# td-kwj-zp2023/webgpu-msm-twisted-edwards

Measured on AMD Instinct MI355X. Metric: MSMs/sec at n=2^20 Twisted-Edwards BLS12 (pipelined throughput = 1000/ms_per_step; single-MSM latency in latency_ms), higher is better.
Workload: dtype u32

## Files before the change

webgpu-msm-twisted-edwards_amd/csrc/kernels.hip.hpp:

```cpp
#pragma once
#include <hip/hip_runtime.h>
#include "curve.hpp"
#include "scalar_form.hpp"

namespace te {

#define TE_BATCH_MAX 8
struct batch_ptrs { const uint4* p[TE_BATCH_MAX]; };
struct batch_slabs { uint32_t s[TE_BATCH_MAX]; };

struct digits_params {
  uint32_t half[10];
  uint32_t zero_digit;
  uint32_t sc_stride;
  uint32_t n, nst;
  int num_windows;
  int w_first, w_step, nw_local;
  uint32_t half_code, logS, P, CH, chunk_len;
};

struct pnt_slot { uint4 q[8]; };
template <bool MONT = false>
__device__ __forceinline__ void prep_points_block(uint32_t blk, uint4* __restrict__ lds, const uint4* __restrict__ pts, pnt_slot* __restrict__ recs, uint32_t n) {
  const uint32_t t = threadIdx.x, base = blk * 256u;
  const bool active = t < 256u;
  const uint32_t pieces_in = (n - base < 256u ? n - base : 256u) * 4u;
// ... 424 lines not shown
__device__ __forceinline__ bool l2_piece_of_block(uint32_t bx, const uint32_t* __restrict__ pc, uint32_t P, uint32_t overflow_pieces, uint32_t* sm, uint32_t* pj, uint32_t& p, uint32_t& j) {
  if (bx < P) { p = bx; j = 0u; return true; }
  const uint32_t t = threadIdx.x, x = bx - P;
  if (x >= overflow_pieces) return false;
  const uint32_t c = t < P ? pc[t] : 0u;
  const uint32_t ov = c ? (c + TE_L2_CAP - 1u) / TE_L2_CAP - 1u : 0u;
  uint32_t tot;
  const uint32_t ex = block_excl_scan(ov, sm, tot);
  if (x >= tot) return false;
  if (x >= ex && x < ex + ov) { pj[0] = t; pj[1] = x - ex + 1u; }
  __syncthreads();
  p = pj[0]; j = pj[1];
  __syncthreads();
  return true;
}

#define TE_COMBINE_SMALL 16u
#define TE_GIANT_RUN 256u
#define TE_SEG_INVALID 0xffffffffu
#define TE_HIST_COPIES 32u
struct plan_args {
  const uint32_t* part_start; const uint32_t* part_count; const uint32_t* seg_part_base;
  uint32_t *bucket_start, *bucket_cursor, *seg_base, *seg_bucket, *seg_lenv, *size_hist, *split_list;
  uint32_t* split_count;
  uint32_t* chunk_list;
  uint32_t seg_len, cap_w, chunk_cap;
};
struct plan_lds { uint32_t h[1024]; uint32_t sm[17]; uint32_t giant[256 * 3]; uint32_t n_giant; };
__device__ __forceinline__ uint32_t seg_plan_block(uint32_t p, uint32_t k, uint32_t cnt_in, const sort_geom& sg, const plan_args& a, plan_lds& L,
                                                   uint32_t pstart, uint32_t pcount, uint32_t sbase) {
  const uint32_t t = threadIdx.x, P = sg.P, S = sg.S, B = sg.B, seg_len = a.seg_len;
  uint32_t* const h = L.h; uint32_t* const sm = L.sm; uint32_t* const giant = L.giant;
  __syncthreads();
  for (uint32_t j = t; j < 1024u; j += 256u) h[j] = 0u;
  if (t == 0) L.n_giant = 0u;
  const bool mine = t < S;
  const uint32_t g = k * B + p * S + (mine ? t : 0u);
  const uint32_t cnt = mine ? cnt_in : 0u;
  const uint32_t nparts = mine ? max(1u, (cnt + seg_len - 1u) / seg_len) : 0u;
  uint32_t bt, bt2;
  const uint32_t ex = block_excl_scan(cnt, sm, bt);
  const uint32_t ex2 = block_excl_scan(nparts, sm, bt2);
  const uint32_t bs = pstart + ex, sb = sbase + ex2;
  if (mine) {
    a.bucket_start[g] = bs; a.bucket_cursor[g] = bs; a.seg_base[g] = sb;
    if (nparts <= TE_COMBINE_SMALL) {
      for (uint32_t part = 0; part < nparts; part++) {
        const uint32_t len = cnt > part * seg_len ? min(seg_len, cnt - part * seg_len) : 0u;
        a.seg_bucket[sb + part] = g; a.seg_lenv[sb + part] = len;
        atomicAdd(&h[min(len, 1023u)], 1u);
      }
      if (nparts > 1u) a.split_list[atomicAdd(&a.split_count[0], 1u)] = g;
    } else {
      const uint32_t j = atomicAdd(&L.n_giant, 1u);
      giant[3 * j] = g; giant[3 * j + 1] = sb; giant[3 * j + 2] = cnt;
      atomicAdd(&a.split_count[1], 1u);
    }
  }
  {
    const uint32_t first = sbase, used = bt2;
    const uint32_t cap = p + 1u == P ? (k + 1u) * a.cap_w - first : S + pcount / seg_len;
    for (uint32_t j = used + t; j < cap; j += 256u) { a.seg_bucket[first + j] = TE_SEG_INVALID; a.seg_lenv[first + j] = TE_SEG_INVALID; }
  }
  __syncthreads();
  const uint32_t ng = L.n_giant;
  for (uint32_t j = 0; j < ng; j++) {
    const uint32_t gg = giant[3 * j], sb0 = giant[3 * j + 1], c0 = giant[3 * j + 2];
    const uint32_t np = (c0 + seg_len - 1u) / seg_len;
    for (uint32_t part = t; part < np; part += 256u) {
      const uint32_t len = min(seg_len, c0 - part * seg_len);
      a.seg_bucket[sb0 + part] = gg; a.seg_lenv[sb0 + part] = len;
      atomicAdd(&h[min(len, 1023u)], 1u);
      if ((part & (TE_GIANT_RUN - 1u)) == 0) { const uint32_t ci = atomicAdd(&a.split_count[2], 1u); if (ci < a.chunk_cap) { a.chunk_list[2 * ci] = gg; a.chunk_list[2 * ci + 1] = part; } }
    }
  }
  __syncthreads();
  uint32_t* my_hist = a.size_hist + ((k * P + p) % TE_HIST_COPIES) * 1024u;
  for (uint32_t j = t; j < 1024u; j += 256u) if (h[j]) atomicAdd(&my_hist[j], h[j]);
  __syncthreads();
  return ex;
}

struct l2_args {
  const uint16_t* part_keys; const uint32_t* part_idx; const uint32_t* part_start; const uint32_t* part_count;
  uint32_t* bucket_count; uint32_t* sorted;
  uint32_t* part_ticket;
  sort_geom g; plan_args pa;
};
#define TE_L2A_LDS_WORDS (3u * 256u + 32u + TE_L2_LIST)
static_assert(sizeof(plan_lds) <= TE_L2_LIST * 4u, "the plan's LDS fits into the list area");
static_assert(TE_L2_CAP < 65536u, "k_l2_local counts a bucket's positive and negative entries in the halves of one word");
template <bool PK>
__global__ void __launch_bounds__(256, TE_L2_WAVES) k_l2_local(l2_args a) {
  __shared__ uint32_t lds[TE_L2A_LDS_WORDS];
// ... 37 lines not shown
  if (t < g.S) a.bucket_count[gb] = c0;
  const uint32_t ex = seg_plan_block(p, k, c0, g, a.pa, PL, pb, cntp, sbp);
  if (t < g.S) a.pa.bucket_cursor[gb] = pb + ex + c0;
  off_s[t] = ex; off_s[256u + t] = ex + c_pos;
  __syncthreads();
#pragma unroll
  for (int c = 0; c < 5; c++) {
    uint32_t kv[8], iv[8]; piece_group<PK>(r, c, kv, iv);
    const uint32_t e0 = ((uint32_t)c * 256u + t) * 8u;
#pragma unroll
    for (int e = 0; e < 8; e++) {
      const uint32_t pos = e0 + (uint32_t)e;
      if (pos >= head && pos < total) list[atomicAdd(&off_s[(kv[e] & 0x7fffu) + ((kv[e] >> 15) << 8)], 1u)] = iv[e] | ((kv[e] >> 15) << 31);
    }
  }
  __syncthreads();
  uint32_t* out = a.sorted + (size_t)k * g.n + pb;
  for (uint32_t s = t; s < cntp; s += 256u) out[s] = list[s];
}

#define TE_ORDER_REGS 32u
__device__ __forceinline__ void order_scatter_block(uint32_t ob, uint32_t nob, uint32_t* __restrict__ lds, const uint32_t* __restrict__ lenv, uint32_t ids,
                                                    const uint32_t* __restrict__ size_hist, uint32_t* __restrict__ rel_cursor,
                                                    uint32_t* __restrict__ order, uint32_t* __restrict__ num_segments, uint32_t max_len) {
  uint32_t* const h = lds; uint32_t* const base = lds + 1024; uint32_t* const sm = lds + 2048;
  const uint32_t per = (ids + nob - 1) / nob;
  const uint32_t lo = min(ids, ob * per), hi = min(ids, lo + per);
  const bool in_regs = per <= TE_ORDER_REGS * 256u;
  uint32_t lv[TE_ORDER_REGS];
  if (in_regs) {
#pragma unroll
    for (uint32_t j = 0; j < TE_ORDER_REGS; j++) { const uint32_t g = lo + j * 256u + threadIdx.x; lv[j] = g < hi ? lenv[g] : TE_SEG_INVALID; }
  }
  for (uint32_t j = threadIdx.x; j < 1024u; j += 256u) h[j] = 0;
  {
    uint32_t run = 0;
    for (uint32_t c = (1023u - min(max_len, 1023u)) >> 8; c < 4u; c++) {
      const uint32_t s = 1023u - (c * 256u + threadIdx.x);
      uint32_t part[TE_HIST_COPIES];
#pragma unroll
      for (uint32_t r = 0; r < TE_HIST_COPIES; r++) part[r] = size_hist[r * 1024u + s];
      uint32_t cnt_s = 0;
#pragma unroll
      for (uint32_t r = 0; r < TE_HIST_COPIES; r++) cnt_s += part[r];
      uint32_t bt;
      const uint32_t ex = block_excl_scan(cnt_s, sm, bt);
      base[s] = run + ex;
      run += bt;
    }
    if (ob == 0 && threadIdx.x == 0) *num_segments = run;
  }
  __syncthreads();
  if (in_regs) {
#pragma unroll
    for (uint32_t j = 0; j < TE_ORDER_REGS; j++) if (lv[j] != TE_SEG_INVALID) atomicAdd(&h[min(lv[j], 1023u)], 1u);
  } else {
    for (uint32_t g = lo + threadIdx.x; g < hi; g += 256u) { const uint32_t l = lenv[g]; if (l != TE_SEG_INVALID) atomicAdd(&h[min(l, 1023u)], 1u); }
  }
  __syncthreads();
  for (uint32_t j = threadIdx.x; j < 1024u; j += 256u) { base[j] += h[j] ? atomicAdd(&rel_cursor[j], h[j]) : 0u; h[j] = 0; }
  __syncthreads();
  if (in_regs) {
#pragma unroll
    for (uint32_t j = 0; j < TE_ORDER_REGS; j++) {
      if (lv[j] == TE_SEG_INVALID) continue;
      const uint32_t sz = min(lv[j], 1023u);
      order[base[sz] + atomicAdd(&h[sz], 1u)] = lo + j * 256u + threadIdx.x;
    }
  } else {
    for (uint32_t g = lo + threadIdx.x; g < hi; g += 256u) {
      const uint32_t l = lenv[g];
      if (l == TE_SEG_INVALID) continue;
      const uint32_t sz = min(l, 1023u);
      order[base[sz] + atomicAdd(&h[sz], 1u)] = g;
    }
  }
}

#define TE_PLACE_LDS_WORDS (4u * 256u + TE_L2_LIST + TE_L2_LIST / 4u + 2u + 17u)
template <bool PK>
__device__ __forceinline__ void l2_place_piece(uint32_t p, uint32_t k, uint32_t a0, uint32_t b0, uint32_t* __restrict__ lds,
                                               const uint16_t* __restrict__ part_keys, const uint32_t* __restrict__ part_idx,
                                               uint32_t* __restrict__ bucket_cursor, uint32_t* __restrict__ sorted, const sort_geom& g) {
  uint32_t* const cnt_s = lds; uint32_t* const lex_s = lds + 256; uint32_t* const off_s = lds + 512; uint32_t* const gbase_s = lds + 768;
  uint32_t* const list = lds + 1024;
  uint8_t* const list_b = reinterpret_cast<uint8_t*>(list + TE_L2_LIST);
  uint32_t* const sm = list + TE_L2_LIST + TE_L2_LIST / 4u + 2u;
  const uint32_t t = threadIdx.x, len = b0 - a0;
  const uint16_t* keys_row = part_keys + (size_t)k * g.nst; const uint32_t* idx_row = part_idx + (size_t)k * g.nst;
  uint32_t* out = sorted + (size_t)k * g.n;
  cnt_s[t] = 0u;
  __syncthreads();
  piece_regs r; uint32_t head, total;
  load_piece<PK>(keys_row, idx_row, a0, b0, t, true, r, head, total);
#pragma unroll
  for (int c = 0; c < 5; c++) {
    uint32_t kv[8], iv[8]; piece_group<PK>(r, c, kv, iv);
// ... 9 lines not shown
  }
  __syncthreads();
  off_s[t] = lex_s[t];
  gbase_s[t] -= lex_s[t];
  __syncthreads();
#pragma unroll
  for (int c = 0; c < 5; c++) {
    uint32_t kv[8], iv[8]; piece_group<PK>(r, c, kv, iv);
    const uint32_t e0 = ((uint32_t)c * 256u + t) * 8u;
#pragma unroll
    for (int e = 0; e < 8; e++) {
      const uint32_t pos = e0 + (uint32_t)e;
      if (pos >= head && pos < total) {
        const uint32_t b = kv[e] & 0x7fffu;
        const uint32_t slot = atomicAdd(&off_s[b], 1u);
        list[slot] = iv[e] | ((kv[e] >> 15) << 31); list_b[slot] = (uint8_t)b;
      }
    }
  }
  __syncthreads();
  for (uint32_t s = t; s < len; s += 256u) out[gbase_s[list_b[s]] + s] = list[s];
}

struct order_args { const uint32_t* lenv; uint32_t ids; const uint32_t* size_hist; uint32_t* rel_cursor; uint32_t* order; uint32_t* num_segments; uint32_t order_cols, max_len; };
template <bool PK>
__global__ void __launch_bounds__(256, TE_L2_WAVES) k_l2_place_order(const uint16_t* __restrict__ part_keys, const uint32_t* __restrict__ part_idx,
                                                           const uint32_t* __restrict__ part_start, const uint32_t* __restrict__ part_count,
                                                           uint32_t* __restrict__ bucket_cursor, uint32_t* __restrict__ sorted, sort_geom g, order_args oa) {
  __shared__ uint32_t lds[TE_PLACE_LDS_WORDS];
  if (blockIdx.x < oa.order_cols) {
    order_scatter_block(blockIdx.y * oa.order_cols + blockIdx.x, gridDim.y * oa.order_cols, lds, oa.lenv, oa.ids, oa.size_hist, oa.rel_cursor, oa.order, oa.num_segments, oa.max_len);
    return;
  }
  const uint32_t k = gridDim.y - 1u - blockIdx.y;
  const uint32_t px = blockIdx.x - oa.order_cols, extra = gridDim.x - oa.order_cols - g.P, bx = px < extra ? g.P + px : px - extra;
  const uint32_t* pc = part_count + k * g.P;
  uint32_t p, j;
  if (!l2_piece_of_block(bx, pc, g.P, bx < g.P ? 0u : part_count[gridDim.y * g.P + k], lds, lds + 32, p, j)) return;
  const uint32_t cntp = pc[p], pb = part_start[k * g.P + p];
  if (cntp <= TE_L2_CAP) return;
  const uint32_t a0 = pb + j * TE_L2_CAP;
  l2_place_piece<PK>(p, k, a0, min(pb + cntp, a0 + TE_L2_CAP), lds, part_keys, part_idx, bucket_cursor, sorted, g);
}

template <int N> struct geo {
  static constexpr uint32_t PW = 4u * N;
  static constexpr uint32_t PQ = PW / 4u;
  static constexpr uint32_t RW = N == 9 ? 27u : 4u * N;
  static constexpr uint32_t SQ = N == 9 ? 8u : N;
  static constexpr uint32_t LQ = (RW + 3u) / 4u;
};
template <int N> struct rec_slot { uint4 q[geo<N>::SQ]; };
static_assert(sizeof(rec_slot<9>) == sizeof(pnt_slot) && sizeof(rec_slot<14>) == 224, "record slots");

// ... 65 lines not shown
#pragma unroll
  for (int j = 0; j < 14; j++) { r.hm.v[j] = w[j]; r.hp.v[j] = w[14 + j]; r.dt.v[j] = w[28 + j]; }
  return r;
}
__device__ __forceinline__ void store_pnt_aff377(rec_aff377* dst, const pnt_aff377& r) {
#pragma unroll
  for (int j = 0; j < 14; j++) { dst->w[j] = r.hm.v[j]; dst->w[14 + j] = r.hp.v[j]; dst->w[28 + j] = r.dt.v[j]; }
}
template <int N, int RK> struct rec_kind;
template <int N> struct rec_kind<N, 0> {
  using slot = rec_slot<N>; using pnt = pnt_t<N>;
  static __device__ __forceinline__ pnt load(const slot* __restrict__ recs, uint32_t e) { return load_pnt<N>(recs, e); }
};
template <> struct rec_kind<14, 1> {
  using slot = rec_aff377; using pnt = pnt_aff377;
  static __device__ __forceinline__ pnt load(const slot* __restrict__ recs, uint32_t e) { return load_pnt_aff377(recs, e); }
};

struct __attribute__((aligned(4))) idx4 { uint32_t v[4]; };
#define TE_CLK_SLOTS 64u
#define TE_IDX_STRIP 16u
template <int N, int RK = 0>
__global__ void __attribute__((amdgpu_flat_work_group_size(1, 256), amdgpu_waves_per_eu(N == 9 ? 3 : 2, N == 9 ? 3 : 2))) k_accumulate(const typename rec_kind<N, RK>::slot* __restrict__ recs, const uint32_t* __restrict__ sorted,
                                                    const uint32_t* __restrict__ bucket_start, const uint32_t* __restrict__ bucket_count,
                                                    const uint32_t* __restrict__ seg_base, const uint32_t* __restrict__ seg_bucket,
                                                    const uint32_t* __restrict__ seg_lenv, const uint32_t* __restrict__ order,
                                                    const uint32_t* __restrict__ num_segments, ete_t<N>* __restrict__ buckets,
                                                    ete_t<N>* __restrict__ seg_out, uint32_t n, uint32_t logB, uint32_t seg_len, uint32_t ids, uint32_t onto,
                                                    uint32_t win_per_msm, batch_slabs slabs, unsigned long long* __restrict__ clk) {
  __shared__ __attribute__((aligned(16))) uint32_t idx_strip[256 * TE_IDX_STRIP];
  using RT = rec_kind<N, RK>; using P = typename RT::pnt;
  unsigned long long* const slot = clk ? clk + (blockIdx.x & (TE_CLK_SLOTS - 1u)) : nullptr;
  const unsigned long long t0_wall = clk ? (unsigned long long)wall_clock64() : 0ull, t0_core = clk ? (unsigned long long)clock64() : 0ull;
  if (clk && threadIdx.x == 0) atomicMax(slot, ~t0_wall);
  const uint32_t gid = blockIdx.x * 256u + threadIdx.x;
  if (gid >= (order ? *num_segments : ids)) return;
  const uint32_t sgm = order ? order[gid] : gid;
  const uint32_t g = seg_bucket[sgm];
  if (g == TE_SEG_INVALID) return;
  const uint32_t k = g >> logB;
  recs += (size_t)slabs.s[k / win_per_msm] * n;
  const uint32_t part = sgm - seg_base[g];
  const uint32_t cnt = seg_lenv[sgm];
  const uint32_t* lst = sorted + (size_t)k * n + bucket_start[g] + part * seg_len;
  ete_t<N> acc = (onto && part == 0u) ? load_ete<N>(buckets + g) : ete_identity_t<N>();
  bool flipped = false;
  if (cnt) {
    const uint32_t last = cnt - 1u;
    uint32_t j0 = 0;
    uint32_t e = lst[0], e_n = lst[min(1u, last)];
    const uint32_t e_2 = lst[min(2u, last)], e_3 = lst[min(3u, last)];
    P cur = RT::load(recs, e);
    if (!(onto && part == 0u)) {
      flipped = (e >> 31) != 0u;
      const bool ends = cnt <= 2u;
      if (cnt >= 2u) {
        const P second = pnt_cneg(RT::load(recs, e_n), ((e_n ^ e) >> 31) != 0u);
        e = e_2; e_n = e_3;
        const P first = cur;
        cur = RT::load(recs, e);
        acc = ete_from_pair<true>(first, second, ends && flipped);
        j0 = 2;
      } else {
        acc = ete_from_pnt<true>(cur, flipped);
        j0 = 1;
      }
    }
    uint32_t* const strip = idx_strip + threadIdx.x * TE_IDX_STRIP;
    auto refill = [&](uint32_t pos) {
      const idx4* src = reinterpret_cast<const idx4*>(lst + pos);
      idx4* dst = reinterpret_cast<idx4*>(strip);
#pragma unroll
      for (uint32_t h = 0; h < TE_IDX_STRIP / 4u; h += 2u) {
        const idx4 v0 = src[h], v1 = src[h + 1u];
        dst[h] = v0; dst[h + 1u] = v1;
      }
// ... 13 lines not shown
        const uint2 e_nn = *reinterpret_cast<const uint2*>(strip + (pn & (TE_IDX_STRIP - 1u)));
        rec_b = RT::load(recs, e_n);
        sign_to(e);
        uv = ete_open<N>(ete_madd_raw(uv, cur));
        __builtin_amdgcn_sched_barrier(0);
        cur = RT::load(recs, e_nn.x);
        sign_to(e_n);
        uv = ete_open<N>(ete_madd_raw(uv, rec_b));
        e = e_nn.x; e_n = e_nn.y;
      }
      {
        const bool two = j + 1u < cnt;
        rec_b = RT::load(recs, two ? e_n : e);
        sign_to(e);
        acc = ete_madd_raw<true>(uv, cur, !two && flipped);
        if (two) {
          uv = ete_open<N>(acc);
          sign_to(e_n);
          acc = ete_madd_raw<true>(uv, rec_b, flipped);
        }
      }
    }
  }
  const bool whole = bucket_count[g] <= seg_len;
  store_ete<N>(whole ? buckets + g : seg_out + sgm, acc);
  if (clk && (uint32_t)__lane_id() == (uint32_t)__ffsll((long long)__ballot(1)) - 1u) {
    const unsigned long long t1_wall = (unsigned long long)wall_clock64(), t1_core = (unsigned long long)clock64();
    atomicMax(slot + TE_CLK_SLOTS, t1_wall);
    atomicAdd(slot + 2u * TE_CLK_SLOTS, t1_core - t0_core); atomicAdd(slot + 3u * TE_CLK_SLOTS, t1_wall - t0_wall);
  }
}

template <int N> struct sum_job_t {
  const ete_t<N>* in; ete_t<N>* out;
  uint32_t n_out;
  uint32_t K, inner;
  uint32_t in_per_window, out_per_window;
};
template <int N> struct sum_jobs_t { sum_job_t<N> j[4]; };
template <int N> __device__ __forceinline__ ete_t<N> pair_swap(const ete_t<N>& a) {
  ete_t<N> r;
#pragma unroll
  for (int i = 0; i < N; i++) {
    r.x.v[i] = (uint32_t)__builtin_amdgcn_mov_dpp((int)a.x.v[i], 0xb1, 0xf, 0xf, true);
    r.y.v[i] = (uint32_t)__builtin_amdgcn_mov_dpp((int)a.y.v[i], 0xb1, 0xf, 0xf, true);
    r.z.v[i] = (uint32_t)__builtin_amdgcn_mov_dpp((int)a.z.v[i], 0xb1, 0xf, 0xf, true);
    r.t.v[i] = (uint32_t)__builtin_amdgcn_mov_dpp((int)a.t.v[i], 0xb1, 0xf, 0xf, true);
  }
// ... 531 lines not shown
```

webgpu-msm-twisted-edwards_amd/csrc/te_msm.hip:

```cpp
#include <hip/hip_runtime.h>
#include <stdint.h>
#include <stdio.h>
#include <stdlib.h>
#include <string.h>
#include <string>
#include <vector>
#include <deque>
#include <algorithm>
#include <functional>
#include <chrono>
#include <thread>
#include <mutex>
#include <condition_variable>
#include <memory>
#include <optional>
#include <type_traits>
#if defined(__x86_64__)
#include <immintrin.h>
#endif

#include "../../include/te_msm.h"
#include "host_tail.hpp"
#include "synth.hpp"
#include "kernels.hip.hpp"
// ... 37 lines not shown
  uint32_t seg_len = 64;
  uint32_t S = 0, logS = 0, P = 0;
  uint32_t packed = 0;
  int rec_kind = 0;
  int scalar_mont = 0;
  int fb_rb = 0, fb_c = 0, fb_W = 0;
};

template <typename T> struct dev_buf {
  T* p = nullptr; size_t cap = 0;
  operator T*() const { return p; }
  void release() { if (p) (void)hipFree(p); p = nullptr; cap = 0; }
};

struct workset_t {
  hipStream_t stream = nullptr, copy_stream = nullptr;
  int hw_queue_class = -1;
  hipEvent_t ev_copy = nullptr, ev_start = nullptr;
  dev_buf<uint8_t> d_recs;
  dev_buf<uint16_t> d_digits, d_part_keys;
  dev_buf<uint32_t> d_part_start, d_part_count, d_part_idx, d_seg_part_base;
  dev_buf<uint32_t> d_bucket_start, d_bucket_cursor, d_sorted;
  dev_buf<uint32_t> d_seg_base, d_seg_bucket, d_seg_lenv, d_order;
  dev_buf<uint32_t> d_split_list, d_chunk_list;
  dev_buf<uint8_t> d_seg_out, d_buckets, d_red[4];
  dev_buf<uint32_t> d_zero; size_t zero_words = 0;
  size_t zero_clean_words = 0;
  uint32_t *d_err = nullptr, *d_num_seg = nullptr, *d_size_hist = nullptr, *d_size_cursor = nullptr, *d_counts1 = nullptr, *d_bucket_count = nullptr;
  uint32_t* d_part_ticket = nullptr;
  uint8_t* d_partials = nullptr;
  uint32_t* h_err = nullptr;
  uint8_t* h_partials = nullptr;
  uint32_t* h_err_dev = nullptr;
  bool rows_on_host = false;
  hipEvent_t ev_done = nullptr;
  hipEvent_t ev_result = nullptr;
  hipEvent_t ev[ST_COUNT + 1] = {};
  plan_t plan; uint64_t n = 0; bool used = false;
  te_sched::slot_t slot;
  std::string job_err;
  int prof_level = 0;
  hipStream_t last_stream = nullptr;
  dev_buf<uint8_t> d_in_points, d_in_scalars;
  std::vector<hipEvent_t> piece_events;
  uint8_t* h_ring = nullptr; std::vector<hipEvent_t> ring_ev; size_t ring_next = 0;
  uint64_t idle_calls = 0;
  dev_buf<uint32_t> d_fb_remap;
  uint32_t* d_fb_fill = nullptr;
  const void* fb_scalars = nullptr; uint64_t fb_n = 0;
  int slab = -1;
  bool slab_run = false;
  const uint8_t* recs_last = nullptr;
  te_bases* bound = nullptr;
  int pt_rc = 0; int64_t pt_index = -1; int pt_reason = 0;
  dev_buf<uint8_t> d_batch_rows;
  dev_buf<uint32_t> d_in_idx;
  template <typename WS, typename F> static void each_buffer(WS& ws, F&& f) {
    f(ws.d_recs); f(ws.d_digits); f(ws.d_part_keys); f(ws.d_part_start); f(ws.d_part_count); f(ws.d_part_idx); f(ws.d_seg_part_base);
    f(ws.d_bucket_start); f(ws.d_bucket_cursor); f(ws.d_sorted); f(ws.d_seg_base); f(ws.d_seg_bucket); f(ws.d_seg_lenv); f(ws.d_order);
    f(ws.d_split_list); f(ws.d_chunk_list); f(ws.d_seg_out); f(ws.d_buckets); for (auto& b : ws.d_red) f(b);
    f(ws.d_zero); f(ws.d_in_points); f(ws.d_in_scalars); f(ws.d_fb_remap); f(ws.d_batch_rows); f(ws.d_in_idx);
  }
};
constexpr int TE_MAX_WINDOWS = 64;
constexpr size_t Z_KEEP = 4;
constexpr size_t Z_ENTRIES = 2;
constexpr size_t Z_CLOCK = 8;
static_assert(Z_KEEP + 4 <= Z_CLOCK && Z_ENTRIES % 2 == 0 && Z_ENTRIES + 2 <= Z_KEEP, "flag words");
constexpr size_t Z_ROWS = Z_CLOCK + 4 * 2 * TE_CLK_SLOTS, Z_HIST = Z_ROWS + (size_t)TE_MAX_WINDOWS * TE_MAX_ROW_BYTES / 4, Z_CURSOR = Z_HIST + 1024 * TE_HIST_COPIES, Z_END = Z_CURSOR + 1024;

struct gpu_t {
  int device = 0;
  int w_first = 0, w_step = 1;
  workset_t ws[TE_MSM_WORKSETS];
  int last_ws = 0;
  int wall_clock_khz = 0;
  int in_flight = 0;
  bool queues_probed = false;
  struct rec_slab_t { const void* src = nullptr; uint64_t n = 0; int curve = 0; uint8_t* d = nullptr; size_t cap = 0; int users = 0;
                      uint32_t pending = 0; hipEvent_t ev[TE_MSM_WORKSETS] = {};
                      int run_users = 0; bool converted = false; hipEvent_t conv_ev = nullptr; };
  std::vector<rec_slab_t> slabs;
// ... 177 lines not shown
  const seq_sizes sz = sizes_for(p, n);
  const size_t nd = (size_t)p.nw * p.nst + 64, wb = sz.wb, ab = sizes_of(p.curve).acc;
  int rc = 0;
  if (need_recs && (rc = make_room(ctx, ws.d_recs, (size_t)n * sizes_of(p.curve).rec * (size_t)p.batch))) return rc;
  if ((rc = make_room(ctx, ws.d_digits, nd))) return rc;
  if ((rc = make_room(ctx, ws.d_sorted, nd))) return rc;
  {
    const size_t c1 = (size_t)p.nw * p.CH * p.P;
    ws.zero_words = Z_END + c1 + wb + (size_t)p.nw * p.P + 64;
    { const uint32_t* before = ws.d_zero; if ((rc = make_room(ctx, ws.d_zero, ws.zero_words))) return rc; if (ws.d_zero != before) ws.zero_clean_words = 0; }
    ws.d_err = ws.d_zero; ws.d_num_seg = ws.d_zero + Z_KEEP; ws.d_size_hist = ws.d_zero + Z_HIST; ws.d_size_cursor = ws.d_zero + Z_CURSOR;
    ws.d_partials = reinterpret_cast<uint8_t*>(ws.d_zero + Z_ROWS);
    ws.d_counts1 = ws.d_zero + Z_END; ws.d_bucket_count = ws.d_counts1 + c1; ws.d_part_ticket = ws.d_bucket_count + wb;
    ws.d_fb_fill = ws.d_part_ticket + (size_t)p.nw * p.P;
  }
  if (p.fb_rb && (rc = make_room(ctx, ws.d_fb_remap, nd))) return rc;
  if ((rc = make_room(ctx, ws.d_bucket_start, wb))) return rc;
  if ((rc = make_room(ctx, ws.d_bucket_cursor, wb))) return rc;
  if ((rc = make_room(ctx, ws.d_seg_part_base, (size_t)p.nw * p.P))) return rc;
  const size_t smax = sz.smax + 16;
  if ((rc = make_room(ctx, ws.d_order, smax))) return rc;
  if ((rc = make_room(ctx, ws.d_seg_bucket, smax))) return rc;
  if ((rc = make_room(ctx, ws.d_seg_lenv, smax))) return rc;
  if ((rc = make_room(ctx, ws.d_seg_out, smax * ab))) return rc;
  if ((rc = make_room(ctx, ws.d_seg_base, wb + 1))) return rc;
  if ((rc = make_room(ctx, ws.d_split_list, wb + 1))) return rc;
  if ((rc = make_room(ctx, ws.d_chunk_list, 2 * sz.chunk_cap(16)))) return rc;
  if ((rc = make_room(ctx, ws.d_part_start, (size_t)p.nw * p.P))) return rc;
  if ((rc = make_room(ctx, ws.d_buckets, wb * ab))) return rc;
  if ((rc = make_room(ctx, ws.d_part_count, (size_t)p.nw * p.P + (size_t)p.nw))) return rc;
  if ((rc = make_room(ctx, ws.d_part_keys, p.packed ? 8 : nd))) return rc;
  if ((rc = make_room(ctx, ws.d_part_idx, nd))) return rc;
  for (int k = 0; k < 4; k++) if ((rc = make_room(ctx, ws.d_red[k], (wb / (k % 2 ? 4 : 2) + 1) * ab))) return rc;
  return 0;
}

template <int LO, int HI, typename F> void with_window_bits(int c, F&& f) {
  if constexpr (LO < HI) { if (c != LO) return with_window_bits<LO + 1, HI>(c, f); }
  f(std::integral_constant<int, LO>{});
}

template <int C, int FORM> void launch_digits(const te::batch_ptrs& sc, int batch, uint16_t* dg, const te::digits_params& prm, uint32_t* err, uint32_t* counts1, hipStream_t s) {
  hipLaunchKernelGGL((te::k_digits<C, FORM>), dim3((prm.nst + TE_DIG_BLOCK - 1u) / TE_DIG_BLOCK, batch), dim3(TE_DIG_THREADS), 0, s, sc, dg, prm, err, counts1);
}
static_assert(TE_BATCH_MAX == TE_MSM_MAX_BATCH, "batch tables");
template <int C, int FORM> void launch_digits_ragged(const void* sc, const te::ragged_tab& tab, int batch, uint16_t* dg, const te::digits_params& prm, uint32_t* err, uint32_t* counts1, hipStream_t s) {
// ... 112 lines not shown
        if (bls()) {
          const uint32_t per_row = (n32 + 511u) / 512u;
          hipLaunchKernelGGL(te::k_part_scatter_prep377, dim3(sblocks + rows * per_row), dim3(512), 0, stream, sa, sblocks, tab, row_slab,
                             reinterpret_cast<te::rec_slot<14>*>(recs_out()), n32, per_row, rows * per_row);
        } else {
          const uint32_t per_row = (n32 + 255u) / 256u;
          hipLaunchKernelGGL(te::k_part_scatter_prep, dim3(sblocks + rows * per_row), dim3(512), 0, stream, sa, sblocks, tab, row_slab,
                             reinterpret_cast<te::pnt_slot*>(recs_out()), n32, per_row, rows * per_row);
        }
      } else if (idx) {
        hipLaunchKernelGGL(te::k_part_scatter_indexed, dim3(p.CH, p.nw), dim3(512), 0, stream, sa, te::index_args{idx, idx_count, idx_pos, ws.d_err});
      } else {
        hipLaunchKernelGGL(te::k_part_scatter, dim3(p.CH, p.nw), dim3(512), 0, stream, sa);
      }
    }
    mark(ST_BSORT);
    if (p.nw > 0) {
      const uint32_t l2_blocks = p.P + n32 / TE_L2_CAP + 1u;
      te::l2_args la;
      la.part_keys = ws.d_part_keys; la.part_idx = ws.d_part_idx; la.part_start = ws.d_part_start; la.part_count = ws.d_part_count;
      la.bucket_count = ws.d_bucket_count; la.sorted = ws.d_sorted; la.part_ticket = ws.d_part_ticket; la.g = sg;
      la.pa.part_start = ws.d_part_start; la.pa.part_count = ws.d_part_count; la.pa.seg_part_base = ws.d_seg_part_base;
      la.pa.bucket_start = ws.d_bucket_start; la.pa.bucket_cursor = ws.d_bucket_cursor; la.pa.seg_base = ws.d_seg_base; la.pa.seg_bucket = ws.d_seg_bucket;
      la.pa.seg_lenv = ws.d_seg_lenv; la.pa.size_hist = ws.d_size_hist; la.pa.split_list = ws.d_split_list; la.pa.split_count = ws.d_num_seg + 1;
      la.pa.chunk_list = ws.d_chunk_list; la.pa.seg_len = p.seg_len; la.pa.cap_w = cap_w; la.pa.chunk_cap = chunk_cap();
      if (p.packed) hipLaunchKernelGGL(te::k_l2_local<true>, dim3(l2_blocks, p.nw), dim3(256), 0, stream, la);
      else hipLaunchKernelGGL(te::k_l2_local<false>, dim3(l2_blocks, p.nw), dim3(256), 0, stream, la);
      te::order_args oa;
      oa.lenv = ws.d_seg_lenv; oa.ids = smax(); oa.size_hist = ws.d_size_hist; oa.rel_cursor = ws.d_size_cursor; oa.order = ws.d_order; oa.num_segments = ws.d_num_seg;
      {
        const uint32_t by_regs = (smax() + TE_ORDER_REGS * 256u * (uint32_t)p.nw - 1u) / (TE_ORDER_REGS * 256u * (uint32_t)p.nw);
        oa.order_cols = std::min(64u, std::max(by_regs, (uint32_t)std::max(1, 128 / p.nw)));
      }
      oa.max_len = std::min(p.seg_len, 1023u);
      if (p.packed)
        hipLaunchKernelGGL(te::k_l2_place_order<true>, dim3(oa.order_cols + l2_blocks, p.nw), dim3(256), 0, stream, ws.d_part_keys, ws.d_part_idx, ws.d_part_start,
                           ws.d_part_count, ws.d_bucket_cursor, ws.d_sorted, sg, oa);
      else
        hipLaunchKernelGGL(te::k_l2_place_order<false>, dim3(oa.order_cols + l2_blocks, p.nw), dim3(256), 0, stream, ws.d_part_keys, ws.d_part_idx, ws.d_part_start,
                           ws.d_part_count, ws.d_bucket_cursor, ws.d_sorted, sg, oa);
    }
    mark(ST_ORDER);
    return 0;
  }

  bool bls() const { return p.curve == TE_MSM_CURVE_BLS12_377_G1; }

  template <int N, int RK> int accumulate_t() {
    mark(ST_ACCUM);
    if (p.nw > 0) {
      const uint32_t n32 = this->n32(), smax = this->smax();
      const uint32_t* order = ctx->opt_sort ? ws.d_order : nullptr;
      using slot_t = typename te::rec_kind<N, RK>::slot;
      hipLaunchKernelGGL((te::k_accumulate<N, RK>), dim3((smax + 255) / 256), dim3(256), 0, stream, reinterpret_cast<const slot_t*>(bound ? bound : recs_out()), ws.d_sorted,
                         ws.d_bucket_start, ws.d_bucket_count, ws.d_seg_base, ws.d_seg_bucket, ws.d_seg_lenv, order, ws.d_num_seg,
                         reinterpret_cast<te::ete_t<N>*>(ws.d_buckets.p), reinterpret_cast<te::ete_t<N>*>(ws.d_seg_out.p), n32, p.logB, p.seg_len, smax, onto ? 1u : 0u,
                         ragged ? (uint32_t)p.nw : (uint32_t)p.nw1, ragged ? te::batch_slabs{} : slabs(),
                         prof ? reinterpret_cast<unsigned long long*>(ws.d_zero + Z_CLOCK) : nullptr);
    }
    return 0;
  }
  int accumulate() { return bls() ? (p.rec_kind == 1 ? accumulate_t<14, 1>() : accumulate_t<14, 0>()) : accumulate_t<9, 0>(); }

  template <int N> int combine_t() {
    if (p.nw <= 0) return 0;
    using E = te::ete_t<N>;
    hipLaunchKernelGGL(te::k_seg_combine_all<N>, dim3(256 + 1024), dim3(256), 0, stream, ws.d_split_list, ws.d_num_seg + 1, ws.d_chunk_list,
                       ws.d_bucket_count, ws.d_seg_base, reinterpret_cast<E*>(ws.d_seg_out.p), reinterpret_cast<E*>(ws.d_buckets.p), p.seg_len, chunk_cap(), 256u,
                       ws.d_bucket_start, ws.d_bucket_cursor);
    return 0;
  }
  int combine() { return bls() ? combine_t<14>() : combine_t<9>(); }

  template <int N> int reduce_t() {
    if (p.nw > 0) {
      using E = te::ete_t<N>;
      const uint32_t w0 = p.dw[0], w1 = p.dw[1], w2 = p.dw[2], w3 = p.dw[3];
      const uint32_t L = 1u << (w0 + w1), H = 1u << (w2 + w3);
      struct chain_t { const E* cur; uint32_t n, r; E* buf[2]; int pp; };
// ... 2580 lines not shown
int64_t te_msm_debug_read(te_ctx* ctx, const char* stage, void* dst, uint64_t cap) {
  device_guard restore_callers_device;
  if (!ctx || !stage || !dst) return TE_MSM_EINVAL;
  drain_workers(ctx);
  gpu_t& d = ctx->devs[0];
  workset_t& ws = d.ws[d.last_ws];
  if (!ws.used) return set_err(ctx, TE_MSM_ESTATE, "no run yet");
  const plan_t& p = ws.plan; const uint64_t n = ws.n;
  const void* src = nullptr; uint64_t bytes = 0;
  if (ws.zero_clean_words && (!strcmp(stage, "bucket_count") || !strcmp(stage, "num_segments") || !strcmp(stage, "partials")))
    return set_err(ctx, TE_MSM_ESTATE, "this stage lives in the block that is cleared behind an MSM's read-back: set option prezero = 0 before the run to keep it");
  if (!strcmp(stage, "records")) {
    if (!ws.recs_last) return set_err(ctx, TE_MSM_ESTATE, "the last run gathered from a bound point set: the work set holds no records of its own");
    src = ws.recs_last; bytes = n * sizes_of(p.curve).rec;
  }
  else if (!strcmp(stage, "digits")) { src = ws.d_digits; bytes = (uint64_t)p.nw * p.nst * 2; }
  else if (!strcmp(stage, "bucket_count")) { src = ws.d_bucket_count; bytes = (uint64_t)p.nw * p.B * 4; }
  else if (!strcmp(stage, "bucket_start")) { src = ws.d_bucket_start; bytes = (uint64_t)p.nw * p.B * 4; }
  else if (!strcmp(stage, "sorted")) { src = ws.d_sorted; bytes = (uint64_t)p.nw * n * 4; }
  else if (!strcmp(stage, "num_segments")) { src = ws.d_num_seg; bytes = 4; }
  else if (!strcmp(stage, "seg_bucket")) { src = ws.d_seg_bucket; bytes = ((uint64_t)p.nw * p.B + (uint64_t)p.nw * (n / p.seg_len)) * 4; }
  else if (!strcmp(stage, "seg_len")) { src = ws.d_seg_lenv; bytes = ((uint64_t)p.nw * p.B + (uint64_t)p.nw * (n / p.seg_len)) * 4; }
  else if (!strcmp(stage, "order")) { src = ws.d_order; bytes = ((uint64_t)p.nw * p.B + (uint64_t)p.nw * (n / p.seg_len)) * 4; }
  else if (!strcmp(stage, "part_start")) { src = ws.d_part_start; bytes = (uint64_t)p.nw * p.P * 4; }
  else if (!strcmp(stage, "part_count")) { src = ws.d_part_count; bytes = (uint64_t)p.nw * p.P * 4; }
  else if (!strcmp(stage, "part_keys") && !p.packed) { src = ws.d_part_keys; bytes = (uint64_t)p.nw * p.nst * 2; }
  else if (!strcmp(stage, "part_idx") && !p.packed) { src = ws.d_part_idx; bytes = (uint64_t)p.nw * p.nst * 4; }
  else if (!strcmp(stage, "part_keys") || !strcmp(stage, "part_idx")) {
    const bool want_keys = stage[5] == 'k';
    const uint64_t words = (uint64_t)p.nw * p.nst;
    std::vector<uint32_t> pk(words);
    HIP_TRY(ctx, hipSetDevice(d.device));
    HIP_TRY(ctx, hipDeviceSynchronize());
    HIP_TRY(ctx, hipMemcpy(pk.data(), ws.d_part_idx, words * 4, hipMemcpyDeviceToHost));
    uint64_t out_bytes = words * (want_keys ? 2 : 4);
    if (out_bytes > cap) out_bytes = cap;
    if (want_keys) { uint16_t* o = static_cast<uint16_t*>(dst); for (uint64_t i = 0; i < out_bytes / 2; i++) o[i] = (uint16_t)(((pk[i] >> 23) & 0xffu) | ((pk[i] >> 31) << 15)); }
    else { uint32_t* o = static_cast<uint32_t*>(dst); for (uint64_t i = 0; i < out_bytes / 4; i++) o[i] = pk[i] & 0x7fffffu; }
    return (int64_t)out_bytes;
  }
  else if (!strcmp(stage, "buckets")) { src = ws.d_buckets; bytes = (uint64_t)p.nw * p.B * sizes_of(p.curve).acc; }
  else if (!strcmp(stage, "partials")) { src = ws.d_partials; bytes = (uint64_t)p.W * sizes_of(p.curve).row; }
  else return set_err(ctx, TE_MSM_EINVAL, "unknown stage");
  if (bytes > cap) bytes = cap;
  HIP_TRY(ctx, hipSetDevice(d.device));
  HIP_TRY(ctx, hipDeviceSynchronize());
// ... 6 lines not shown
```

Measured before the change: 1152.

## Pack per-segment metadata into 16-byte descriptors scattered in schedule order

The planning pass now builds a 16-byte descriptor per segment holding list position, bucket id, segment id, and count with first-part and whole-bucket flags. The order scatter copies each descriptor into schedule order, so the accumulate kernel reads one contiguous 16-byte record. This replaces the order lookup plus dependent gathers of seg_bucket, seg_base, seg_lenv, bucket_start and bucket_count. The cost is extra descriptor writes in the plan and order kernels and two more buffers, while the old per-field arrays are still written.

```diff
diff --git a/webgpu-msm-twisted-edwards_amd/csrc/kernels.hip.hpp b/webgpu-msm-twisted-edwards_amd/csrc/kernels.hip.hpp
--- a/webgpu-msm-twisted-edwards_amd/csrc/kernels.hip.hpp
+++ b/webgpu-msm-twisted-edwards_amd/csrc/kernels.hip.hpp
@@ -2,6 +2,7 @@
 #include <hip/hip_runtime.h>
 #include "curve.hpp"
 #include "scalar_form.hpp"
+#include "seg_desc.hpp"
 
 namespace te {
 
@@ -472,11 +473,12 @@
 struct plan_args {
   const uint32_t* part_start; const uint32_t* part_count; const uint32_t* seg_part_base;
   uint32_t *bucket_start, *bucket_cursor, *seg_base, *seg_bucket, *seg_lenv, *size_hist, *split_list;
+  te_seg::desc* seg_desc;
   uint32_t* split_count;
   uint32_t* chunk_list;
   uint32_t seg_len, cap_w, chunk_cap;
 };
-struct plan_lds { uint32_t h[1024]; uint32_t sm[17]; uint32_t giant[256 * 3]; uint32_t n_giant; };
+struct plan_lds { uint32_t h[1024]; uint32_t sm[17]; uint32_t giant[256 * 4]; uint32_t n_giant; };
 __device__ __forceinline__ uint32_t seg_plan_block(uint32_t p, uint32_t k, uint32_t cnt_in, const sort_geom& sg, const plan_args& a, plan_lds& L,
                                                    uint32_t pstart, uint32_t pcount, uint32_t sbase) {
   const uint32_t t = threadIdx.x, P = sg.P, S = sg.S, B = sg.B, seg_len = a.seg_len;
@@ -498,28 +500,30 @@
       for (uint32_t part = 0; part < nparts; part++) {
         const uint32_t len = cnt > part * seg_len ? min(seg_len, cnt - part * seg_len) : 0u;
         a.seg_bucket[sb + part] = g; a.seg_lenv[sb + part] = len;
+        a.seg_desc[sb + part] = te_seg::compose(g, bs, cnt, sb, part, seg_len);
         atomicAdd(&h[min(len, 1023u)], 1u);
       }
       if (nparts > 1u) a.split_list[atomicAdd(&a.split_count[0], 1u)] = g;
     } else {
       const uint32_t j = atomicAdd(&L.n_giant, 1u);
-      giant[3 * j] = g; giant[3 * j + 1] = sb; giant[3 * j + 2] = cnt;
+      giant[4 * j] = g; giant[4 * j + 1] = sb; giant[4 * j + 2] = cnt; giant[4 * j + 3] = bs;
       atomicAdd(&a.split_count[1], 1u);
     }
   }
   {
     const uint32_t first = sbase, used = bt2;
     const uint32_t cap = p + 1u == P ? (k + 1u) * a.cap_w - first : S + pcount / seg_len;
-    for (uint32_t j = used + t; j < cap; j += 256u) { a.seg_bucket[first + j] = TE_SEG_INVALID; a.seg_lenv[first + j] = TE_SEG_INVALID; }
+    for (uint32_t j = used + t; j < cap; j += 256u) { a.seg_bucket[first + j] = TE_SEG_INVALID; a.seg_lenv[first + j] = TE_SEG_INVALID; a.seg_desc[first + j] = te_seg::invalid(); }
   }
   __syncthreads();
   const uint32_t ng = L.n_giant;
   for (uint32_t j = 0; j < ng; j++) {
-    const uint32_t gg = giant[3 * j], sb0 = giant[3 * j + 1], c0 = giant[3 * j + 2];
+    const uint32_t gg = giant[4 * j], sb0 = giant[4 * j + 1], c0 = giant[4 * j + 2], bs0 = giant[4 * j + 3];
     const uint32_t np = (c0 + seg_len - 1u) / seg_len;
     for (uint32_t part = t; part < np; part += 256u) {
       const uint32_t len = min(seg_len, c0 - part * seg_len);
       a.seg_bucket[sb0 + part] = gg; a.seg_lenv[sb0 + part] = len;
+      a.seg_desc[sb0 + part] = te_seg::compose(gg, bs0, c0, sb0, part, seg_len);
       atomicAdd(&h[min(len, 1023u)], 1u);
       if ((part & (TE_GIANT_RUN - 1u)) == 0) { const uint32_t ci = atomicAdd(&a.split_count[2], 1u); if (ci < a.chunk_cap) { a.chunk_list[2 * ci] = gg; a.chunk_list[2 * ci + 1] = part; } }
     }
@@ -603,7 +607,8 @@
 #define TE_ORDER_REGS 32u
 __device__ __forceinline__ void order_scatter_block(uint32_t ob, uint32_t nob, uint32_t* __restrict__ lds, const uint32_t* __restrict__ lenv, uint32_t ids,
                                                     const uint32_t* __restrict__ size_hist, uint32_t* __restrict__ rel_cursor,
-                                                    uint32_t* __restrict__ order, uint32_t* __restrict__ num_segments, uint32_t max_len) {
+                                                    uint32_t* __restrict__ order, uint32_t* __restrict__ num_segments, uint32_t max_len,
+                                                    const te_seg::desc* __restrict__ seg_desc, te_seg::desc* __restrict__ sched_desc) {
   uint32_t* const h = lds; uint32_t* const base = lds + 1024; uint32_t* const sm = lds + 2048;
   const uint32_t per = (ids + nob - 1) / nob;
   const uint32_t lo = min(ids, ob * per), hi = min(ids, lo + per);
@@ -646,14 +651,16 @@
     for (uint32_t j = 0; j < TE_ORDER_REGS; j++) {
       if (lv[j] == TE_SEG_INVALID) continue;
       const uint32_t sz = min(lv[j], 1023u);
-      order[base[sz] + atomicAdd(&h[sz], 1u)] = lo + j * 256u + threadIdx.x;
+      const uint32_t g = lo + j * 256u + threadIdx.x, pos = base[sz] + atomicAdd(&h[sz], 1u);
+      order[pos] = g; sched_desc[pos] = seg_desc[g];
     }
   } else {
     for (uint32_t g = lo + threadIdx.x; g < hi; g += 256u) {
       const uint32_t l = lenv[g];
       if (l == TE_SEG_INVALID) continue;
       const uint32_t sz = min(l, 1023u);
-      order[base[sz] + atomicAdd(&h[sz], 1u)] = g;
+      const uint32_t pos = base[sz] + atomicAdd(&h[sz], 1u);
+      order[pos] = g; sched_desc[pos] = seg_desc[g];
     }
   }
 }
@@ -709,14 +716,14 @@
   for (uint32_t s = t; s < len; s += 256u) out[gbase_s[list_b[s]] + s] = list[s];
 }
 
-struct order_args { const uint32_t* lenv; uint32_t ids; const uint32_t* size_hist; uint32_t* rel_cursor; uint32_t* order; uint32_t* num_segments; uint32_t order_cols, max_len; };
+struct order_args { const uint32_t* lenv; uint32_t ids; const uint32_t* size_hist; uint32_t* rel_cursor; uint32_t* order; uint32_t* num_segments; uint32_t order_cols, max_len; const te_seg::desc* seg_desc; te_seg::desc* sched_desc; };
 template <bool PK>
 __global__ void __launch_bounds__(256, TE_L2_WAVES) k_l2_place_order(const uint16_t* __restrict__ part_keys, const uint32_t* __restrict__ part_idx,
                                                            const uint32_t* __restrict__ part_start, const uint32_t* __restrict__ part_count,
                                                            uint32_t* __restrict__ bucket_cursor, uint32_t* __restrict__ sorted, sort_geom g, order_args oa) {
   __shared__ uint32_t lds[TE_PLACE_LDS_WORDS];
   if (blockIdx.x < oa.order_cols) {
-    order_scatter_block(blockIdx.y * oa.order_cols + blockIdx.x, gridDim.y * oa.order_cols, lds, oa.lenv, oa.ids, oa.size_hist, oa.rel_cursor, oa.order, oa.num_segments, oa.max_len);
+    order_scatter_block(blockIdx.y * oa.order_cols + blockIdx.x, gridDim.y * oa.order_cols, lds, oa.lenv, oa.ids, oa.size_hist, oa.rel_cursor, oa.order, oa.num_segments, oa.max_len, oa.seg_desc, oa.sched_desc);
     return;
   }
   const uint32_t k = gridDim.y - 1u - blockIdx.y;
@@ -828,11 +835,9 @@
 #define TE_IDX_STRIP 16u
 template <int N, int RK = 0>
 __global__ void __attribute__((amdgpu_flat_work_group_size(1, 256), amdgpu_waves_per_eu(N == 9 ? 3 : 2, N == 9 ? 3 : 2))) k_accumulate(const typename rec_kind<N, RK>::slot* __restrict__ recs, const uint32_t* __restrict__ sorted,
-                                                    const uint32_t* __restrict__ bucket_start, const uint32_t* __restrict__ bucket_count,
-                                                    const uint32_t* __restrict__ seg_base, const uint32_t* __restrict__ seg_bucket,
-                                                    const uint32_t* __restrict__ seg_lenv, const uint32_t* __restrict__ order,
+                                                    const te_seg::desc* __restrict__ descs, uint32_t scheduled,
                                                     const uint32_t* __restrict__ num_segments, ete_t<N>* __restrict__ buckets,
-                                                    ete_t<N>* __restrict__ seg_out, uint32_t n, uint32_t logB, uint32_t seg_len, uint32_t ids, uint32_t onto,
+                                                    ete_t<N>* __restrict__ seg_out, uint32_t n, uint32_t logB, uint32_t ids, uint32_t onto,
                                                     uint32_t win_per_msm, batch_slabs slabs, unsigned long long* __restrict__ clk) {
   __shared__ __attribute__((aligned(16))) uint32_t idx_strip[256 * TE_IDX_STRIP];
   using RT = rec_kind<N, RK>; using P = typename RT::pnt;
@@ -840,16 +845,17 @@
   const unsigned long long t0_wall = clk ? (unsigned long long)wall_clock64() : 0ull, t0_core = clk ? (unsigned long long)clock64() : 0ull;
   if (clk && threadIdx.x == 0) atomicMax(slot, ~t0_wall);
   const uint32_t gid = blockIdx.x * 256u + threadIdx.x;
-  if (gid >= (order ? *num_segments : ids)) return;
-  const uint32_t sgm = order ? order[gid] : gid;
-  const uint32_t g = seg_bucket[sgm];
-  if (g == TE_SEG_INVALID) return;
+  if (gid >= (scheduled ? *num_segments : ids)) return;
+  const te_seg::desc sd = descs[gid];
+  const uint32_t g = sd.g;
+  if (g == te_seg::kInvalid) return;
   const uint32_t k = g >> logB;
   recs += (size_t)slabs.s[k / win_per_msm] * n;
-  const uint32_t part = sgm - seg_base[g];
-  const uint32_t cnt = seg_lenv[sgm];
-  const uint32_t* lst = sorted + (size_t)k * n + bucket_start[g] + part * seg_len;
-  ete_t<N> acc = (onto && part == 0u) ? load_ete<N>(buckets + g) : ete_identity_t<N>();
+  const uint32_t cnt = te_seg::count(sd);
+  const bool part0 = te_seg::first_part(sd);
+  const uint32_t* lst = sorted + (size_t)k * n + sd.pos;
+  ete_t<N>* const dst = te_seg::whole(sd) ? buckets + g : seg_out + sd.id;
+  ete_t<N> acc = (onto && part0) ? load_ete<N>(buckets + g) : ete_identity_t<N>();
   bool flipped = false;
   if (cnt) {
     const uint32_t last = cnt - 1u;
@@ -857,7 +863,7 @@
     uint32_t e = lst[0], e_n = lst[min(1u, last)];
     const uint32_t e_2 = lst[min(2u, last)], e_3 = lst[min(3u, last)];
     P cur = RT::load(recs, e);
-    if (!(onto && part == 0u)) {
+    if (!(onto && part0)) {
       flipped = (e >> 31) != 0u;
       const bool ends = cnt <= 2u;
       if (cnt >= 2u) {
@@ -917,8 +923,7 @@
       }
     }
   }
-  const bool whole = bucket_count[g] <= seg_len;
-  store_ete<N>(whole ? buckets + g : seg_out + sgm, acc);
+  store_ete<N>(dst, acc);
   if (clk && (uint32_t)__lane_id() == (uint32_t)__ffsll((long long)__ballot(1)) - 1u) {
     const unsigned long long t1_wall = (unsigned long long)wall_clock64(), t1_core = (unsigned long long)clock64();
     atomicMax(slot + TE_CLK_SLOTS, t1_wall);
diff --git a/webgpu-msm-twisted-edwards_amd/csrc/seg_desc.hpp b/webgpu-msm-twisted-edwards_amd/csrc/seg_desc.hpp
--- /dev/null
+++ b/webgpu-msm-twisted-edwards_amd/csrc/seg_desc.hpp
@@ -0,0 +1,50 @@
+#pragma once
+#include <stdint.h>
+
+#if defined(__HIPCC__)
+#include <hip/hip_runtime.h>
+#ifndef TE_HD
+#define TE_HD __host__ __device__ __forceinline__
+#endif
+#else
+#ifndef TE_HD
+#define TE_HD inline
+#endif
+#endif
+
+namespace te_seg {
+
+struct __attribute__((aligned(16))) desc { uint32_t pos, g, id, cw; };
+static_assert(sizeof(desc) == 16, "one 16-byte access per descriptor");
+
+constexpr uint32_t kInvalid = 0xffffffffu;
+constexpr uint32_t kCountMask = 0x3fffffffu, kFirst = 1u << 30, kWhole = 1u << 31;
+constexpr uint32_t kMaxSegLen = 1000000u;
+static_assert(kMaxSegLen <= kCountMask, "a segment's count leaves the two flag bits free");
+
+TE_HD uint32_t part_len(uint32_t count, uint32_t part, uint32_t seg_len) {
+  const uint32_t off = part * seg_len;
+  if (off >= count) return 0u;
+  const uint32_t rest = count - off;
+  return rest < seg_len ? rest : seg_len;
+}
+TE_HD uint32_t parts_of(uint32_t count, uint32_t seg_len) {
+  const uint32_t np = (uint32_t)(((uint64_t)count + seg_len - 1u) / seg_len);
+  return np ? np : 1u;
+}
+TE_HD desc compose(uint32_t g, uint32_t bucket_start, uint32_t bucket_count, uint32_t seg_base, uint32_t part, uint32_t seg_len) {
+  desc d;
+  d.pos = bucket_start + part * seg_len;
+  d.g = g;
+  d.id = seg_base + part;
+  d.cw = part_len(bucket_count, part, seg_len) | (part == 0u ? kFirst : 0u) | (bucket_count <= seg_len ? kWhole : 0u);
+  return d;
+}
+TE_HD desc invalid() { desc d; d.pos = 0u; d.g = kInvalid; d.id = kInvalid; d.cw = 0u; return d; }
+
+TE_HD bool valid(const desc& d) { return d.g != kInvalid; }
+TE_HD uint32_t count(const desc& d) { return d.cw & kCountMask; }
+TE_HD bool first_part(const desc& d) { return (d.cw & kFirst) != 0u; }
+TE_HD bool whole(const desc& d) { return (d.cw & kWhole) != 0u; }
+
+}
diff --git a/webgpu-msm-twisted-edwards_amd/csrc/te_msm.hip b/webgpu-msm-twisted-edwards_amd/csrc/te_msm.hip
--- a/webgpu-msm-twisted-edwards_amd/csrc/te_msm.hip
+++ b/webgpu-msm-twisted-edwards_amd/csrc/te_msm.hip
@@ -83,6 +83,7 @@
   dev_buf<uint32_t> d_part_start, d_part_count, d_part_idx, d_seg_part_base;
   dev_buf<uint32_t> d_bucket_start, d_bucket_cursor, d_sorted;
   dev_buf<uint32_t> d_seg_base, d_seg_bucket, d_seg_lenv, d_order;
+  dev_buf<te_seg::desc> d_seg_desc, d_sched_desc;
   dev_buf<uint32_t> d_split_list, d_chunk_list;
   dev_buf<uint8_t> d_seg_out, d_buckets, d_red[4];
   dev_buf<uint32_t> d_zero; size_t zero_words = 0;
@@ -119,6 +120,7 @@
   template <typename WS, typename F> static void each_buffer(WS& ws, F&& f) {
     f(ws.d_recs); f(ws.d_digits); f(ws.d_part_keys); f(ws.d_part_start); f(ws.d_part_count); f(ws.d_part_idx); f(ws.d_seg_part_base);
     f(ws.d_bucket_start); f(ws.d_bucket_cursor); f(ws.d_sorted); f(ws.d_seg_base); f(ws.d_seg_bucket); f(ws.d_seg_lenv); f(ws.d_order);
+    f(ws.d_seg_desc); f(ws.d_sched_desc);
     f(ws.d_split_list); f(ws.d_chunk_list); f(ws.d_seg_out); f(ws.d_buckets); for (auto& b : ws.d_red) f(b);
     f(ws.d_zero); f(ws.d_in_points); f(ws.d_in_scalars); f(ws.d_fb_remap); f(ws.d_batch_rows); f(ws.d_in_idx);
   }
@@ -342,6 +344,8 @@
   if ((rc = make_room(ctx, ws.d_order, smax))) return rc;
   if ((rc = make_room(ctx, ws.d_seg_bucket, smax))) return rc;
   if ((rc = make_room(ctx, ws.d_seg_lenv, smax))) return rc;
+  if ((rc = make_room(ctx, ws.d_seg_desc, smax))) return rc;
+  if ((rc = make_room(ctx, ws.d_sched_desc, smax))) return rc;
   if ((rc = make_room(ctx, ws.d_seg_out, smax * ab))) return rc;
   if ((rc = make_room(ctx, ws.d_seg_base, wb + 1))) return rc;
   if ((rc = make_room(ctx, ws.d_split_list, wb + 1))) return rc;
@@ -500,12 +504,13 @@
       la.bucket_count = ws.d_bucket_count; la.sorted = ws.d_sorted; la.part_ticket = ws.d_part_ticket; la.g = sg;
       la.pa.part_start = ws.d_part_start; la.pa.part_count = ws.d_part_count; la.pa.seg_part_base = ws.d_seg_part_base;
       la.pa.bucket_start = ws.d_bucket_start; la.pa.bucket_cursor = ws.d_bucket_cursor; la.pa.seg_base = ws.d_seg_base; la.pa.seg_bucket = ws.d_seg_bucket;
-      la.pa.seg_lenv = ws.d_seg_lenv; la.pa.size_hist = ws.d_size_hist; la.pa.split_list = ws.d_split_list; la.pa.split_count = ws.d_num_seg + 1;
+      la.pa.seg_lenv = ws.d_seg_lenv; la.pa.seg_desc = ws.d_seg_desc; la.pa.size_hist = ws.d_size_hist; la.pa.split_list = ws.d_split_list; la.pa.split_count = ws.d_num_seg + 1;
       la.pa.chunk_list = ws.d_chunk_list; la.pa.seg_len = p.seg_len; la.pa.cap_w = cap_w; la.pa.chunk_cap = chunk_cap();
       if (p.packed) hipLaunchKernelGGL(te::k_l2_local<true>, dim3(l2_blocks, p.nw), dim3(256), 0, stream, la);
       else hipLaunchKernelGGL(te::k_l2_local<false>, dim3(l2_blocks, p.nw), dim3(256), 0, stream, la);
       te::order_args oa;
       oa.lenv = ws.d_seg_lenv; oa.ids = smax(); oa.size_hist = ws.d_size_hist; oa.rel_cursor = ws.d_size_cursor; oa.order = ws.d_order; oa.num_segments = ws.d_num_seg;
+      oa.seg_desc = ws.d_seg_desc; oa.sched_desc = ws.d_sched_desc;
       {
         const uint32_t by_regs = (smax() + TE_ORDER_REGS * 256u * (uint32_t)p.nw - 1u) / (TE_ORDER_REGS * 256u * (uint32_t)p.nw);
         oa.order_cols = std::min(64u, std::max(by_regs, (uint32_t)std::max(1, 128 / p.nw)));
@@ -528,11 +533,11 @@
     mark(ST_ACCUM);
     if (p.nw > 0) {
       const uint32_t n32 = this->n32(), smax = this->smax();
-      const uint32_t* order = ctx->opt_sort ? ws.d_order : nullptr;
+      const te_seg::desc* descs = ctx->opt_sort ? ws.d_sched_desc : ws.d_seg_desc;
       using slot_t = typename te::rec_kind<N, RK>::slot;
       hipLaunchKernelGGL((te::k_accumulate<N, RK>), dim3((smax + 255) / 256), dim3(256), 0, stream, reinterpret_cast<const slot_t*>(bound ? bound : recs_out()), ws.d_sorted,
-                         ws.d_bucket_start, ws.d_bucket_count, ws.d_seg_base, ws.d_seg_bucket, ws.d_seg_lenv, order, ws.d_num_seg,
-                         reinterpret_cast<te::ete_t<N>*>(ws.d_buckets.p), reinterpret_cast<te::ete_t<N>*>(ws.d_seg_out.p), n32, p.logB, p.seg_len, smax, onto ? 1u : 0u,
+                         descs, ctx->opt_sort ? 1u : 0u, ws.d_num_seg,
+                         reinterpret_cast<te::ete_t<N>*>(ws.d_buckets.p), reinterpret_cast<te::ete_t<N>*>(ws.d_seg_out.p), n32, p.logB, smax, onto ? 1u : 0u,
                          ragged ? (uint32_t)p.nw : (uint32_t)p.nw1, ragged ? te::batch_slabs{} : slabs(),
                          prof ? reinterpret_cast<unsigned long long*>(ws.d_zero + Z_CLOCK) : nullptr);
     }
@@ -3159,6 +3164,8 @@
   else if (!strcmp(stage, "seg_bucket")) { src = ws.d_seg_bucket; bytes = ((uint64_t)p.nw * p.B + (uint64_t)p.nw * (n / p.seg_len)) * 4; }
   else if (!strcmp(stage, "seg_len")) { src = ws.d_seg_lenv; bytes = ((uint64_t)p.nw * p.B + (uint64_t)p.nw * (n / p.seg_len)) * 4; }
   else if (!strcmp(stage, "order")) { src = ws.d_order; bytes = ((uint64_t)p.nw * p.B + (uint64_t)p.nw * (n / p.seg_len)) * 4; }
+  else if (!strcmp(stage, "seg_desc")) { src = ws.d_seg_desc; bytes = ((uint64_t)p.nw * p.B + (uint64_t)p.nw * (n / p.seg_len)) * sizeof(te_seg::desc); }
+  else if (!strcmp(stage, "sched_desc")) { src = ws.d_sched_desc; bytes = ((uint64_t)p.nw * p.B + (uint64_t)p.nw * (n / p.seg_len)) * sizeof(te_seg::desc); }
   else if (!strcmp(stage, "part_start")) { src = ws.d_part_start; bytes = (uint64_t)p.nw * p.P * 4; }
   else if (!strcmp(stage, "part_count")) { src = ws.d_part_count; bytes = (uint64_t)p.nw * p.P * 4; }
   else if (!strcmp(stage, "part_keys") && !p.packed) { src = ws.d_part_keys; bytes = (uint64_t)p.nw * p.nst * 2; }
```

Result: no change. 1155 (median of 6 runs) (+0.2%).
